# hangxu0304/DeepReduce

Measured on NVIDIA H100. Metric: ResNet-50 images/sec (whole job, device-timed, max over ranks), higher is better.
Workload: dtype bf16

## Files before the change

### deepreduce_b200/models/fused_bn.py

```python
from __future__ import annotations

import os

import torch
import torch.nn as nn
import torch.nn.functional as F


def enabled() -> bool:
    return os.environ.get("DR_FUSED_BN", "1") != "0"


def _eligible_x(x: torch.Tensor) -> bool:
    return (x.is_cuda and x.dtype == torch.bfloat16 and x.dim() == 4 and x.stride(1) == 1
            and x.is_contiguous(memory_format=torch.channels_last) and x.size(1) % 8 == 0 and x.size(1) <= 8192
            and x.numel() < 2 ** 31 - 1 and x.numel() // x.size(1) > 1)


def _eligible_bn(bn: nn.BatchNorm2d) -> bool:
    return (bn.training and bn.track_running_stats and bn.running_mean is not None and bn.momentum is not None
            and bn.affine)


def eligible(x: torch.Tensor, bn: nn.BatchNorm2d) -> bool:
    return enabled() and _eligible_x(x) and _eligible_bn(bn)


def _stats(x, bn):
    from .. import ops
    bn.num_batches_tracked.add_(1)
    return ops.cuda_module().bn_stats(x, bn.running_mean, bn.running_var, float(bn.momentum), float(bn.eps))


def _grad(go):
    return go.contiguous(memory_format=torch.channels_last)


class _BNReLU(torch.autograd.Function):
    @staticmethod
    def forward(ctx, x, weight, bias, mean, invstd):
        from .. import ops
        y, mask = ops.cuda_module().bn_apply(0, x, [mean, invstd, weight, bias])
        ctx.save_for_backward(x, weight, mean, invstd, mask)
        return y

    @staticmethod
    def backward(ctx, gy):
        from .. import ops
        x, weight, mean, invstd, mask = ctx.saved_tensors
        dx, dw, db = ops.cuda_module().bn_backward(0, _grad(gy), mask, x, [mean, invstd, weight])
        return dx, dw, db, None, None


class _BNAddReLU(torch.autograd.Function):

    @staticmethod
    def forward(ctx, x, weight, bias, mean, invstd, z, wz, bz, mz, iz):
        from .. import ops
        mod = ops.cuda_module()
        if wz is None:
            o, mask = mod.bn_apply(1, x, [mean, invstd, weight, bias], z)
            ctx.save_for_backward(x, weight, mean, invstd, mask)
        else:
            o, mask = mod.bn_apply(2, x, [mean, invstd, weight, bias], z, [mz, iz, wz, bz])
            ctx.save_for_backward(x, weight, mean, invstd, mask, z, wz, mz, iz)
        ctx.has_bn_z = wz is not None
        return o

    @staticmethod
    def backward(ctx, go):
        from .. import ops
        mod = ops.cuda_module()
        saved = ctx.saved_tensors
        x, weight, mean, invstd, mask = saved[:5]
        if not ctx.has_bn_z:
            dx, dw, db, g = mod.bn_backward(1, _grad(go), mask, x, [mean, invstd, weight])
            return dx, dw, db, None, None, g, None, None, None, None
        z, wz, mz, iz = saved[5:]
        dx, dw, db, dz, dwz, dbz = mod.bn_backward(2, _grad(go), mask, x, [mean, invstd, weight], z, [mz, iz, wz])
        return dx, dw, db, None, None, dz, dwz, dbz, None, None


class _BNReLUMaxPool(torch.autograd.Function):

    @staticmethod
    def forward(ctx, x, weight, bias, mean, invstd):
        from .. import ops
        out, codes = ops.cuda_module().bn_apply_pool(x, [mean, invstd, weight, bias])
        ctx.save_for_backward(x, weight, mean, invstd, codes)
        return out

    @staticmethod
    def backward(ctx, go):
        from .. import ops
        x, weight, mean, invstd, codes = ctx.saved_tensors
        dx, dw, db = ops.cuda_module().bn_backward(3, _grad(go), codes, x, [mean, invstd, weight])
        return dx, dw, db, None, None


def _stem_pool(pool: nn.Module) -> bool:
    if type(pool) is not nn.MaxPool2d:
        return False
    pair = lambda v: tuple(v) if isinstance(v, (tuple, list)) else (v, v)
    return (pair(pool.kernel_size) == (3, 3) and pair(pool.stride) == (2, 2) and pair(pool.padding) == (1, 1)
            and pair(pool.dilation) == (1, 1) and not pool.ceil_mode and not pool.return_indices)


def bn_relu_maxpool(x: torch.Tensor, bn: nn.BatchNorm2d, pool: nn.MaxPool2d) -> torch.Tensor:
    if not (eligible(x, bn) and _stem_pool(pool)):
        return pool(F.relu(bn(x), inplace=True))
    mean, invstd = _stats(x, bn)
    return _BNReLUMaxPool.apply(x, bn.weight, bn.bias, mean, invstd)


def bn_relu(x: torch.Tensor, bn: nn.BatchNorm2d) -> torch.Tensor:
    if not eligible(x, bn):
        return F.relu(bn(x), inplace=True)
    mean, invstd = _stats(x, bn)
    return _BNReLU.apply(x, bn.weight, bn.bias, mean, invstd)


def bn_add_relu(x: torch.Tensor, bn: nn.BatchNorm2d, idt: torch.Tensor) -> torch.Tensor:
    if not (eligible(x, bn) and idt.dtype == x.dtype and idt.shape == x.shape and idt.stride() == x.stride()):
        return F.relu(bn(x) + idt, inplace=True)
    mean, invstd = _stats(x, bn)
    return _BNAddReLU.apply(x, bn.weight, bn.bias, mean, invstd, idt, None, None, None, None)


def bn_bn_add_relu(x: torch.Tensor, bn: nn.BatchNorm2d, xd: torch.Tensor, bnd: nn.BatchNorm2d) -> torch.Tensor:
    if not (eligible(x, bn) and eligible(xd, bnd) and xd.shape == x.shape and xd.stride() == x.stride()):
        return F.relu(bn(x) + bnd(xd), inplace=True)
    md, id_ = _stats(xd, bnd)
    mean, invstd = _stats(x, bn)
    return _BNAddReLU.apply(x, bn.weight, bn.bias, mean, invstd, xd, bnd.weight, bnd.bias, md, id_)
```

### deepreduce_b200/models/resnet.py

```python
from __future__ import annotations

import torch.nn as nn
import torch.nn.functional as F

from .fused_bn import bn_add_relu, bn_bn_add_relu, bn_relu, bn_relu_maxpool


class _BasicCifar(nn.Module):
    def __init__(self, inp, out, stride):
        super().__init__()
        self.conv1 = nn.Conv2d(inp, out, 3, stride, 1, bias=False)
        self.bn1 = nn.BatchNorm2d(out)
        self.conv2 = nn.Conv2d(out, out, 3, 1, 1, bias=False)
        self.bn2 = nn.BatchNorm2d(out)
        self.pad = None
        if stride != 1 or inp != out:
            self.pad = (out - inp, stride)

    def forward(self, x):
        y = F.relu(self.bn1(self.conv1(x)))
        y = self.bn2(self.conv2(y))
        if self.pad is not None:
            extra, s = self.pad
            x = F.pad(x[:, :, ::s, ::s], (0, 0, 0, 0, extra // 2, extra - extra // 2))
# ... 20 lines not shown
        return self.fc(x)


def resnet20(num_classes: int = 10) -> ResNetCifar:
    return ResNetCifar(3, num_classes)


class _Bottleneck(nn.Module):
    expansion = 4

    def __init__(self, inp, width, stride, downsample):
        super().__init__()
        out = width * self.expansion
        self.conv1 = nn.Conv2d(inp, width, 1, bias=False)
        self.bn1 = nn.BatchNorm2d(width)
        self.conv2 = nn.Conv2d(width, width, 3, stride, 1, bias=False)
        self.bn2 = nn.BatchNorm2d(width)
        self.conv3 = nn.Conv2d(width, out, 1, bias=False)
        self.bn3 = nn.BatchNorm2d(out)
        self.downsample = None
        if downsample:
            self.downsample = nn.Sequential(nn.Conv2d(inp, out, 1, stride, bias=False), nn.BatchNorm2d(out))

    def forward(self, x):
        xd = None if self.downsample is None else self.downsample[0](x)
        y = bn_relu(self.conv1(x), self.bn1)
        y = bn_relu(self.conv2(y), self.bn2)
        y = self.conv3(y)
        if xd is None:
            return bn_add_relu(y, self.bn3, x)
        return bn_bn_add_relu(y, self.bn3, xd, self.downsample[1])


class ResNet(nn.Module):
    def __init__(self, blocks=(3, 4, 6, 3), num_classes: int = 1000):
        super().__init__()
        self.conv1 = nn.Conv2d(3, 64, 7, 2, 3, bias=False)
        self.bn1 = nn.BatchNorm2d(64)
        self.maxpool = nn.MaxPool2d(3, 2, 1)
        stages, inp = [], 64
        for i, (n, width) in enumerate(zip(blocks, (64, 128, 256, 512))):
            for j in range(n):
                stride = 2 if (j == 0 and i > 0) else 1
                stages.append(_Bottleneck(inp, width, stride, downsample=(j == 0)))
                inp = width * 4
        self.layers = nn.Sequential(*stages)
        self.fc = nn.Linear(inp, num_classes)
        for m in self.modules():
            if isinstance(m, nn.Conv2d):
                nn.init.kaiming_normal_(m.weight, mode="fan_out", nonlinearity="relu")

    def forward(self, x):
        x = bn_relu_maxpool(self.conv1(x), self.bn1, self.maxpool)
        x = self.layers(x)
        x = F.adaptive_avg_pool2d(x, 1).flatten(1)
        return self.fc(x)


def resnet50(num_classes: int = 1000) -> ResNet:
    return ResNet((3, 4, 6, 3), num_classes)
```

### deepreduce_b200/ops/csrc/binding.cpp

```cpp
#include <ATen/cuda/CUDAContext.h>
#include <c10/cuda/CUDAGuard.h>
#include <c10/cuda/CUDAStream.h>
#include <torch/extension.h>

#include <condition_variable>
#include <deque>
#include <mutex>
#include <thread>

#include "ops.h"

namespace py = pybind11;
using dr::EngineParams;

#define CHECK_CUDA_T(x) TORCH_CHECK((x).is_cuda() && (x).is_contiguous(), #x " must be a contiguous CUDA tensor")

static cudaStream_t cur_stream() { return at::cuda::getCurrentCUDAStream().stream(); }

static void check_last(const char* what) {
  cudaError_t e = cudaGetLastError();
  TORCH_CHECK(e == cudaSuccess, what, ": ", cudaGetErrorString(e));
}

static torch::Tensor bloom_insert(torch::Tensor idx, int64_t k, int64_t m_bits, int64_t seed) {
// ... 296 lines not shown
              "bn_apply_pool: only kernel 3, stride 2, padding 1, dilation 1, floor mode");
  check_bn_input(x);
  const int64_t N = x.size(0), C = x.size(1), H = x.size(2), W = x.size(3);
  const dr::BnParams px = bn_params(p, C);
  c10::cuda::CUDAGuard g(x.device());
  const dr::PoolGeom pg{(int)H, (int)W, (int)((H - 1) / 2 + 1), (int)((W - 1) / 2 + 1)};
  auto out = torch::empty({N, C, pg.Ho, pg.Wo}, x.options().memory_format(at::MemoryFormat::ChannelsLast));
  auto codes = torch::empty({N * pg.Ho * pg.Wo, C}, x.options().dtype(torch::kUInt8));
  cudaError_t e = dr::launch_bn_apply_pool(x.data_ptr(), px, out.data_ptr(), codes.data_ptr(), (int)N, pg, (int)C,
                                           cur_stream());
  TORCH_CHECK(e == cudaSuccess, "bn_apply_pool: ", cudaGetErrorString(e));
  return {out, codes};
}

static dr::BnParams bn_bwd_params(const std::vector<torch::Tensor>& p, int64_t C) {
  TORCH_CHECK(p.size() == 3, "bn_backward: expected (mean, invstd, weight)");
  const char* names[3] = {"mean", "invstd", "weight"};
  for (int i = 0; i < 3; ++i) check_chan(p[i], C, names[i]);
  return {p[0].data_ptr<float>(), p[1].data_ptr<float>(), p[2].data_ptr<float>(), nullptr};
}

static std::vector<torch::Tensor> bn_backward(int64_t mode, torch::Tensor go, torch::Tensor mask, torch::Tensor x,
                                              std::vector<torch::Tensor> p, c10::optional<torch::Tensor> z,
                                              std::vector<torch::Tensor> pz) {
  TORCH_CHECK(mode >= 0 && mode <= 3, "bn_backward: mode must be 0, 1, 2 or 3");
  check_bn_input(x);
  const int64_t C = x.size(1), rows = x.numel() / C;
  dr::PoolGeom pg{(int)x.size(2), (int)x.size(3), (int)((x.size(2) - 1) / 2 + 1), (int)((x.size(3) - 1) / 2 + 1)};
  const std::vector<int64_t> go_shape =
      mode == 3 ? std::vector<int64_t>{x.size(0), C, pg.Ho, pg.Wo} : x.sizes().vec();
  TORCH_CHECK(go.sizes() == go_shape && go.scalar_type() == torch::kBFloat16 && go.device() == x.device() &&
                  go.is_contiguous(at::MemoryFormat::ChannelsLast),
              "bn_backward: go must be a channels_last bf16 tensor on x's device, of x's shape (mode 3: the pooled "
              "shape)");
  const int64_t mask_numel = mode == 3 ? go.numel() : rows * (C / 8);
  TORCH_CHECK(mask.is_cuda() && mask.scalar_type() == torch::kUInt8 && mask.is_contiguous() &&
                  mask.numel() == mask_numel && mask.device() == x.device(),
              "bn_backward: mask must be bn_apply's mask (mode 3: bn_apply_pool's codes) for x");
  c10::cuda::CUDAGuard guard(x.device());
  int block_y = 0, grid_y = 0;
  dr::bn_row_tree(rows, (int)C, &block_y, &grid_y);
  TORCH_CHECK((int64_t)block_y * grid_y <= rows, "bn_backward: reduction tree wider than the rows");
  const int n_sums = mode == 2 ? 3 : 2;
  auto f32 = x.options().dtype(torch::kFloat32);
  auto sums = torch::empty({n_sums, C}, f32);
  auto staging = grid_y > 1 ? torch::empty({n_sums, grid_y, C}, f32) : torch::Tensor();
  auto dx = torch::empty_like(x), dw = torch::empty({C}, f32), db = torch::empty({C}, f32);
  dr::BnBwd b{};
  b.go = go.data_ptr(); b.mask = mask.data_ptr<uint8_t>(); b.x = x.data_ptr();
  b.px = bn_bwd_params(p, C);
  b.dx = dx.data_ptr(); b.sums = sums.data_ptr<float>(); b.staging = grid_y > 1 ? staging.data_ptr<float>() : nullptr;
  b.dw = dw.data_ptr<float>(); b.db = db.data_ptr<float>();
  b.pool = pg;
  std::vector<torch::Tensor> res{dx, dw, db};
  torch::Tensor g;
  if (mode == 1 || mode == 3) {
    g = torch::empty_like(x);
    b.g = g.data_ptr();
    if (mode == 1) res.push_back(g);
  } else if (mode == 2) {
    TORCH_CHECK(z.has_value(), "bn_backward: mode 2 needs z");
    check_like_x(*z, x, "z");
    b.z = z->data_ptr();
    b.pz = bn_bwd_params(pz, C);
    auto dz = torch::empty_like(x), dwz = torch::empty({C}, f32), dbz = torch::empty({C}, f32);
    b.dz = dz.data_ptr(); b.dwz = dwz.data_ptr<float>(); b.dbz = dbz.data_ptr<float>();
    res.insert(res.end(), {dz, dwz, dbz});
  }
  cudaError_t e = dr::launch_bn_backward((int)mode, b, rows, (int)C, cur_stream());
  TORCH_CHECK(e == cudaSuccess, "bn_backward: ", cudaGetErrorString(e));
  return res;
}
// ... 201 lines not shown

PYBIND11_MODULE(TORCH_EXTENSION_NAME, m) {
  m.def("launch_count", [] { return (int64_t)dr::launch_count(); });
  m.def("bloom_insert", &bloom_insert);
  m.def("bloom_select", &bloom_select);
  m.def("qsgd_encode", &qsgd_encode);
  m.def("qsgd_decode", &qsgd_decode);
  m.def("pack_bits", &pack_bits);
  m.def("unpack_bits", &unpack_bits);
  m.def("polyfit_fit", &polyfit_fit);
  m.def("polyfit_eval", &polyfit_eval);
  m.def("dexp_fit", &dexp_fit);
  m.def("conflict_sets_pick", &conflict_sets_pick);
  m.def("delta_bp128_encode", &delta_bp128_encode);
  m.def("delta_bp128_decode", &delta_bp128_decode);
  m.def("u8_to_nhwc_norm", &u8_to_nhwc_norm);
  m.def("bn_stats", &bn_stats, py::arg("x"), py::arg("running_mean"), py::arg("running_var"), py::arg("momentum"),
        py::arg("eps"), py::arg("torch_kernel") = false);
  m.def("bn_apply", &bn_apply, py::arg("mode"), py::arg("x"), py::arg("p"), py::arg("z") = py::none(),
        py::arg("pz") = std::vector<torch::Tensor>{});
  m.def("bn_apply_pool", &bn_apply_pool, py::arg("x"), py::arg("p"), py::arg("kernel_size") = 3, py::arg("stride") = 2,
        py::arg("padding") = 1, py::arg("dilation") = 1, py::arg("ceil_mode") = false);
  m.def("bn_backward", &bn_backward, py::arg("mode"), py::arg("go"), py::arg("mask"), py::arg("x"), py::arg("p"),
        py::arg("z") = py::none(), py::arg("pz") = std::vector<torch::Tensor>{});
  m.def("rle_runs", &rle_runs);
  m.def("rle_indices", &rle_indices);
  m.def("arena_alloc", &arena_alloc);
  m.def("arena_free", [](int64_t p) { dr::arena_free((void*)p); });
  m.def("arena_export", &arena_export);
  m.def("arena_import", &arena_import);
  m.def("arena_close", [](int64_t p) { dr::arena_close((void*)p); });
  m.def("arena_as_tensor", &arena_as_tensor);
  m.def("enable_peer_access", [](std::vector<int> devices) { return dr::arena_enable_peer_access(devices.data(), (int)devices.size()); });
  m.attr("TILE") = dr::kTile;
  m.attr("ARENA_HDR_WORDS") = dr::kArenaHdrWords;
  m.attr("SLOT_HEADER_WORDS") = dr::kSlotHeaderWords;
  m.attr("HIST_BINS") = dr::kHistBins;
  m.attr("NUM_HIST") = dr::kNumHist;
  m.attr("PH_END") = (int)dr::kPhEnd;

  py::class_<Engine>(m, "Engine")
      .def(py::init<int64_t, int64_t, int64_t, int64_t, int64_t, int64_t, int64_t, int64_t, int64_t, int64_t, int64_t,
                    int64_t, int64_t, int64_t, std::vector<int64_t>, int, int>())
      .def("configure", &Engine::configure)
      .def("set_buffers", &Engine::set_buffers)
      .def("set_poly", &Engine::set_poly)
      .def("set_shard", &Engine::set_shard)
// ... 20 lines not shown
```

### deepreduce_b200/ops/csrc/bn.cu

```cuda
#include <cuda_bf16.h>

#include <algorithm>

#include "common.cuh"
#include "ops.h"

namespace dr {

namespace {

constexpr int kVec = 8;
constexpr int kApplyThreads = 256;
constexpr int kReduceThreads = 128;

struct ChanParams {
  float m[kVec], inv[kVec], w[kVec], b[kVec];
};

__device__ __forceinline__ void load8(const float* __restrict__ p, float* d) {
  const float4 a = __ldg(reinterpret_cast<const float4*>(p));
  const float4 b = __ldg(reinterpret_cast<const float4*>(p) + 1);
  d[0] = a.x; d[1] = a.y; d[2] = a.z; d[3] = a.w;
  d[4] = b.x; d[5] = b.y; d[6] = b.z; d[7] = b.w;
}

__device__ __forceinline__ void load_params(const BnParams& p, int c, ChanParams& o) {
  load8(p.mean + c, o.m);
  load8(p.invstd + c, o.inv);
  load8(p.weight + c, o.w);
  load8(p.bias + c, o.b);
}

__device__ __forceinline__ float bn_elem(float x, float m, float inv, float w, float b) {
  return __fmaf_rn(__fmul_rn(w, __fsub_rn(x, m)), inv, b);
}

__device__ __forceinline__ __nv_bfloat16 relu_bf16(__nv_bfloat16 v) {
  return __bfloat162float(v) <= 0.f ? __float2bfloat16_rn(0.f) : v;
}

template <int kMode>
__global__ void __launch_bounds__(kApplyThreads) bn_apply_kernel(const __nv_bfloat16* __restrict__ x, BnParams px,
                                                                 const __nv_bfloat16* __restrict__ z, BnParams pz,
                                                                 __nv_bfloat16* __restrict__ out,
                                                                 uint8_t* __restrict__ mask, int64_t rows, int C) {
  const int groups = C / kVec;
  const int rows_per_cta = blockDim.x / groups;
  const int rsub = threadIdx.x / groups;
  if (rsub >= rows_per_cta) return;
  const int c = (threadIdx.x % groups) * kVec;
  ChanParams a;
  load_params(px, c, a);
  ChanParams d;
  if (kMode == 2) load_params(pz, c, d);
  const int64_t step = (int64_t)gridDim.x * rows_per_cta;
#pragma unroll 2
  for (int64_t r = (int64_t)blockIdx.x * rows_per_cta + rsub; r < rows; r += step) {
    const int64_t off = r * C + c;
    const uint4 vx = *reinterpret_cast<const uint4*>(x + off);
    uint4 vz = make_uint4(0, 0, 0, 0);
    if (kMode != 0) vz = *reinterpret_cast<const uint4*>(z + off);
// ... 85 lines not shown
  uint4 g[4];
  uint2 code[4];
  int off;
  int nh, nw;
  int sh, sw;
};

__device__ __forceinline__ void pool_gather_codes(PoolGather& q, const uint8_t* __restrict__ codes, const PoolGeom& pg,
                                                  int row, int C, int c, bool valid) {
  const int w = row % pg.W, t = row / pg.W, h = t % pg.H, n = t / pg.H;
  const int ph = h >> 1, pw = w >> 1;
  q.nh = valid ? min((h + 1) / 2 + 1, pg.Ho) - ph : 0;
  q.nw = valid ? min((w + 1) / 2 + 1, pg.Wo) - pw : 0;
  q.sh = h - 2 * ph + 1;
  q.sw = w - 2 * pw + 1;
  q.off = ((n * pg.Ho + ph) * pg.Wo + pw) * C + c;
#pragma unroll
  for (int k = 0; k < 4; ++k) {
    const int a = k >> 1, b = k & 1;
    q.code[k] = a < q.nh && b < q.nw ? *reinterpret_cast<const uint2*>(codes + q.off + (a * pg.Wo + b) * C) : uint2{};
  }
}

__device__ __forceinline__ void pool_gather_grads(PoolGather& q, const __nv_bfloat16* __restrict__ gp,
                                                  const PoolGeom& pg, int C) {
#pragma unroll
  for (int k = 0; k < 4; ++k) {
    const int a = k >> 1, b = k & 1;
    q.g[k] = a < q.nh && b < q.nw ? *reinterpret_cast<const uint4*>(gp + q.off + (a * pg.Wo + b) * C) : uint4{};
  }
}

__device__ __forceinline__ void pool_gather_resolve(const PoolGather& q, uint4& g, unsigned& bits) {
  __nv_bfloat16* hg = reinterpret_cast<__nv_bfloat16*>(&g);
  const bool single = q.nh == 1 && q.nw == 1;
  bits = 0;
#pragma unroll
  for (int i = 0; i < kVec; ++i) {
    float s = 0.f;
    __nv_bfloat16 one = __float2bfloat16_rn(0.f);
    unsigned bit = 0;
#pragma unroll
    for (int k = 0; k < 4; ++k) {
      const int a = k >> 1, b = k & 1;
      const unsigned code = (reinterpret_cast<const uint8_t*>(&q.code[k]))[i];
      if (a < q.nh && b < q.nw && (int)(code & 0x7fu) == (q.sh - 2 * a) * 3 + (q.sw - 2 * b)) {
        const __nv_bfloat16 v = (reinterpret_cast<const __nv_bfloat16*>(&q.g[k]))[i];
        s = __fadd_rn(s, __bfloat162float(v));
        one = v;
        bit = code >> 7;
      }
    }
    hg[i] = single ? one : __float2bfloat16_rn(s);
    bits |= bit << i;
  }
}

__global__ void __launch_bounds__(kApplyThreads) bn_pool_grad_kernel(const __nv_bfloat16* __restrict__ gp,
                                                                     const uint8_t* __restrict__ codes,
                                                                     __nv_bfloat16* __restrict__ g, PoolGeom pg,
                                                                     int64_t rows, int C) {
  const int groups = C / kVec;
  const int rows_per_cta = blockDim.x / groups;
  const int rsub = threadIdx.x / groups;
  if (rsub >= rows_per_cta) return;
  const int c = (threadIdx.x % groups) * kVec;
  const int64_t step = (int64_t)gridDim.x * rows_per_cta;
#pragma unroll 2
  for (int64_t r = (int64_t)blockIdx.x * rows_per_cta + rsub; r < rows; r += step) {
    PoolGather q;
    pool_gather_codes(q, codes, pg, (int)r, C, c, true);
    pool_gather_grads(q, gp, pg, C);
    uint4 v;
    unsigned bits;
    pool_gather_resolve(q, v, bits);
    __nv_bfloat16* hv = reinterpret_cast<__nv_bfloat16*>(&v);
#pragma unroll
    for (int i = 0; i < kVec; ++i)
      if (!((bits >> i) & 1u)) hv[i] = __float2bfloat16_rn(0.f);
    *reinterpret_cast<uint4*>(g + r * C + c) = v;
  }
}

struct RowTree {
  int block_y, grid_y;
  __host__ __device__ int S() const { return block_y * grid_y; }
  __host__ __device__ int loops(int rows) const { return 1 + (rows - 1) / (S() * kLoads); }
  static constexpr int kLoads = 4;
};

constexpr int kStatsThreads = 256;

__device__ __forceinline__ void welford_update(float x, float inv, float valid, float& mean, float& m2n) {
  const float d0 = __fsub_rn(x, mean);
  mean = __fmaf_rn(d0, inv, mean);
// ... 165 lines not shown
}

struct BwdOut {
  float* sums;
  float* dw; float* db; float* dwz; float* dbz;
  float* staging;
};

__device__ __forceinline__ void bwd_store(const BwdOut& o, int k, int c, int C, float v, const float* invstd,
                                         const float* invstd_z) {
  o.sums[k * C + c] = v;
  if (k == 0) {
    o.db[c] = v;
    if (o.dbz) o.dbz[c] = v;
  } else if (k == 1) {
    o.dw[c] = __fmul_rn(v, invstd[c]);
  } else {
    o.dwz[c] = __fmul_rn(v, invstd_z[c]);
  }
}

__device__ __forceinline__ float masked(__nv_bfloat16 go, unsigned bit) { return bit ? __bfloat162float(go) : 0.f; }

template <int kMode>
__global__ void __launch_bounds__(kReduceThreads) bn_bwd_reduce_kernel(const __nv_bfloat16* __restrict__ go,
                                                                       const uint8_t* __restrict__ mask,
                                                                       const __nv_bfloat16* __restrict__ x,
                                                                       const float* __restrict__ mean,
                                                                       const float* __restrict__ invstd,
                                                                       const __nv_bfloat16* __restrict__ z,
                                                                       const float* __restrict__ mean_z,
                                                                       const float* __restrict__ invstd_z,
                                                                       __nv_bfloat16* __restrict__ g_out, BwdOut o,
                                                                       RowTree t, int rows, int C) {
  constexpr int kSums = kMode == 2 ? 3 : 2;
  constexpr int L = RowTree::kLoads;
  extern __shared__ float sh[];
  const int gpc = blockDim.x / t.block_y;
  const int tg = threadIdx.x % gpc, y = threadIdx.x / gpc;
  const int group = blockIdx.x * gpc + tg;
  const bool live = group * kVec < C;
  const int c = live ? group * kVec : 0;
  const int S = t.S();
  float m[kVec], mz[kVec];
#pragma unroll
  for (int i = 0; i < kVec; ++i) {
    m[i] = mean[c + i];
    mz[i] = kMode == 2 ? mean_z[c + i] : 0.f;
  }
  float acc[kSums][L][kVec];
#pragma unroll
  for (int k = 0; k < kSums; ++k)
#pragma unroll
    for (int j = 0; j < L; ++j)
#pragma unroll
      for (int i = 0; i < kVec; ++i) acc[k][j][i] = 0.f;
  const int mgroups = C / kVec;
  int r = blockIdx.y * t.block_y + y;
  const int n_loops = t.loops(rows);
  struct Batch {
    uint4 g[L], x[L], z[L];
    unsigned m[L];
  };
  auto load = [&](Batch& b, int r0) {
#pragma unroll
    for (int j = 0; j < L; ++j) {
      const int rr = r0 + j * S;
      if (live && rr < rows) {
        const int off = rr * C + c;
        b.g[j] = *reinterpret_cast<const uint4*>(go + off);
        b.x[j] = *reinterpret_cast<const uint4*>(x + off);
        if (kMode == 2) b.z[j] = *reinterpret_cast<const uint4*>(z + off);
        b.m[j] = kMode == 3 ? 0u : mask[rr * mgroups + group];
      } else {
        b.g[j] = uint4{}; b.x[j] = uint4{}; b.z[j] = uint4{}; b.m[j] = 0;
      }
    }
  };
  Batch cur;
  load(cur, r);
  for (int it = 0; it < n_loops; ++it) {
    Batch nxt;
    load(nxt, r + L * S);
    const unsigned* mb = cur.m;
#pragma unroll
    for (int j = 0; j < L; ++j) {
      const __nv_bfloat16* hg = reinterpret_cast<const __nv_bfloat16*>(&cur.g[j]);
      const __nv_bfloat16* hx = reinterpret_cast<const __nv_bfloat16*>(&cur.x[j]);
      const __nv_bfloat16* hz = reinterpret_cast<const __nv_bfloat16*>(&cur.z[j]);
      uint4 vo;
      __nv_bfloat16* ho = reinterpret_cast<__nv_bfloat16*>(&vo);
#pragma unroll
      for (int i = 0; i < kVec; ++i) {
        const unsigned bit = (mb[j] >> i) & 1u;
        const float g = kMode == 3 ? __bfloat162float(hg[i]) : masked(hg[i], bit);
        if (kMode == 1) ho[i] = bit ? hg[i] : __float2bfloat16_rn(0.f);
        acc[0][j][i] = __fadd_rn(acc[0][j][i], g);
        acc[1][j][i] = __fmaf_rn(__fsub_rn(__bfloat162float(hx[i]), m[i]), g, acc[1][j][i]);
        if (kMode == 2) acc[2][j][i] = __fmaf_rn(__fsub_rn(__bfloat162float(hz[i]), mz[i]), g, acc[2][j][i]);
      }
      if (kMode == 1 && live && r + j * S < rows) *reinterpret_cast<uint4*>(g_out + (r + j * S) * C + c) = vo;
    }
    cur = nxt;
    r += L * S;
  }
#pragma unroll
  for (int k = 0; k < kSums; ++k) {
#pragma unroll
    for (int i = 0; i < kVec; ++i)
#pragma unroll
      for (int j = 1; j < L; ++j) acc[k][0][i] = __fadd_rn(acc[k][0][i], acc[k][j][i]);
    tree_over_y<kVec>(acc[k][0], sh, y, t.block_y, tg * kVec, gpc * kVec);
  }
  if (y != 0 || !live) return;
#pragma unroll
  for (int k = 0; k < kSums; ++k)
#pragma unroll
    for (int i = 0; i < kVec; ++i) {
      if (t.grid_y > 1) o.staging[((size_t)k * t.grid_y + blockIdx.y) * C + c + i] = acc[k][0][i];
      else bwd_store(o, k, c + i, C, acc[k][0][i], invstd, invstd_z);
    }
}

__global__ void bn_bwd_finalize_kernel(BwdOut o, RowTree t, int n_sums, int C, const float* __restrict__ invstd,
                                       const float* __restrict__ invstd_z) {
  extern __shared__ float sh[];
// ... 18 lines not shown
  float inv[kVec], ww[kVec], sx[kVec];
  load8(mean + c, p.m);
  load8(invstd + c, inv);
  load8(w + c, ww);
  load8(sdy + c, p.sdy);
  load8(sxmu + c, sx);
#pragma unroll
  for (int i = 0; i < kVec; ++i) {
    p.f1[i] = __fmul_rn(__fmul_rn(__fmul_rn(inv[i], inv[i]), sx[i]), norm);
    p.f2[i] = __fmul_rn(ww[i], inv[i]);
  }
}

__device__ __forceinline__ __nv_bfloat16 elemt(float g, float x, const ElemtChan& p, int i, float norm) {
  const float a = __fmaf_rn(-p.sdy[i], norm, g);
  return __float2bfloat16_rn(__fmul_rn(__fmaf_rn(-p.f1[i], __fsub_rn(x, p.m[i]), a), p.f2[i]));
}

struct ElemtArgs {
  const float *mean, *invstd, *weight, *sums;
  const float *mean_z, *invstd_z, *weight_z;
};

template <int kMode>
__global__ void __launch_bounds__(kApplyThreads) bn_bwd_elemt_kernel(const __nv_bfloat16* __restrict__ g_in,
                                                                     const uint8_t* __restrict__ mask,
                                                                     const __nv_bfloat16* __restrict__ x,
                                                                     const __nv_bfloat16* __restrict__ z, ElemtArgs a,
                                                                     __nv_bfloat16* __restrict__ dx,
                                                                     __nv_bfloat16* __restrict__ dz, float norm,
                                                                     int64_t rows, int C) {
  const int groups = C / kVec;
  const int rows_per_cta = blockDim.x / groups;
  const int rsub = threadIdx.x / groups;
  if (rsub >= rows_per_cta) return;
  const int c = (threadIdx.x % groups) * kVec;
  ElemtChan p;
  elemt_params(a.mean, a.invstd, a.weight, a.sums, a.sums + C, norm, c, p);
  ElemtChan q;
  if (kMode == 2) elemt_params(a.mean_z, a.invstd_z, a.weight_z, a.sums, a.sums + 2 * C, norm, c, q);
  const int64_t step = (int64_t)gridDim.x * rows_per_cta;
#pragma unroll 2
  for (int64_t r = (int64_t)blockIdx.x * rows_per_cta + rsub; r < rows; r += step) {
    const int64_t off = r * C + c;
    const uint4 vg = *reinterpret_cast<const uint4*>(g_in + off);
    const unsigned mb = kMode == 1 || kMode == 3 ? 0xffu : mask[r * groups + c / kVec];
    const uint4 vx = *reinterpret_cast<const uint4*>(x + off);
    uint4 vz = make_uint4(0, 0, 0, 0);
    if (kMode == 2) vz = *reinterpret_cast<const uint4*>(z + off);
    const __nv_bfloat16* hg = reinterpret_cast<const __nv_bfloat16*>(&vg);
    const __nv_bfloat16* hx = reinterpret_cast<const __nv_bfloat16*>(&vx);
    const __nv_bfloat16* hz = reinterpret_cast<const __nv_bfloat16*>(&vz);
    uint4 vo, vd;
    __nv_bfloat16* ho = reinterpret_cast<__nv_bfloat16*>(&vo);
    __nv_bfloat16* hd = reinterpret_cast<__nv_bfloat16*>(&vd);
#pragma unroll
    for (int i = 0; i < kVec; ++i) {
      const float g = masked(hg[i], (mb >> i) & 1u);
      ho[i] = elemt(g, __bfloat162float(hx[i]), p, i, norm);
      if (kMode == 2) hd[i] = elemt(g, __bfloat162float(hz[i]), q, i, norm);
    }
    *reinterpret_cast<uint4*>(dx + off) = vo;
    if (kMode == 2) *reinterpret_cast<uint4*>(dz + off) = vd;
  }
}

__global__ void bn_update_stats_kernel(const float* __restrict__ mean, float* __restrict__ var_invstd,
                                       float* __restrict__ running_mean, float* __restrict__ running_var, int C,
// ... 29 lines not shown
  cudaError_t e = rows_grid(bn_apply_kernel<kMode>, rows, C, grid, threads);
  if (e != cudaSuccess) return e;
  count_launch();
  bn_apply_kernel<kMode><<<grid, threads, 0, st>>>(reinterpret_cast<const __nv_bfloat16*>(x), px,
                                                   reinterpret_cast<const __nv_bfloat16*>(z), pz,
                                                   reinterpret_cast<__nv_bfloat16*>(out),
                                                   reinterpret_cast<uint8_t*>(mask), rows, C);
  return cudaGetLastError();
}

int last_pow2(unsigned n) {
  n |= n >> 1; n |= n >> 2; n |= n >> 4; n |= n >> 8; n |= n >> 16;
  return std::max<int>(1, (int)(n - (n >> 1)));
}

RowTree row_tree(int rows, int C) {
  const int block_x = std::min(last_pow2((unsigned)C), 32);
  const int block_y = std::min(last_pow2((unsigned)((rows + 15) / 16)), 512 / block_x);
  int grid_y = std::min((rows + block_y * 16 - 1) / (block_y * 16), 128);
  if (grid_y < 8) grid_y = 1;
  return {block_y, grid_y};
}

template <int kMode>
cudaError_t launch_bwd_reduce(const BnBwd& b, const RowTree& t, const BwdOut& o, int rows, int C, cudaStream_t st) {
  const int groups = C / kVec;
  const int gpc = std::min(groups, std::max(1, kReduceThreads / t.block_y));
  const dim3 grid((groups + gpc - 1) / gpc, t.grid_y);
  const int threads = gpc * t.block_y;
  count_launch();
  bn_bwd_reduce_kernel<kMode><<<grid, threads, threads * kVec * sizeof(float), st>>>(
      reinterpret_cast<const __nv_bfloat16*>(b.go), b.mask, reinterpret_cast<const __nv_bfloat16*>(b.x), b.px.mean,
      b.px.invstd, reinterpret_cast<const __nv_bfloat16*>(b.z), b.pz.mean, b.pz.invstd,
      reinterpret_cast<__nv_bfloat16*>(b.g), o, t, rows, C);
  return cudaGetLastError();
}

template <int kMode>
cudaError_t launch_bwd_elemt(const BnBwd& b, const ElemtArgs& a, int64_t rows, int C, cudaStream_t st) {
  int grid = 0, threads = 0;
  cudaError_t e = rows_grid(bn_bwd_elemt_kernel<kMode>, rows, C, grid, threads);
  if (e != cudaSuccess) return e;
  const float norm = (float)(1.0 / (double)rows);
  count_launch();
  bn_bwd_elemt_kernel<kMode><<<grid, threads, 0, st>>>(
      reinterpret_cast<const __nv_bfloat16*>(kMode == 1 || kMode == 3 ? b.g : b.go), b.mask,
      reinterpret_cast<const __nv_bfloat16*>(b.x), reinterpret_cast<const __nv_bfloat16*>(b.z), a,
      reinterpret_cast<__nv_bfloat16*>(b.dx), reinterpret_cast<__nv_bfloat16*>(b.dz), norm, rows, C);
  return cudaGetLastError();
}

template <int kMode>
cudaError_t launch_backward(const BnBwd& b, int64_t rows64, int C, cudaStream_t st) {
  const int rows = (int)rows64;
  const RowTree t = row_tree(rows, C);
  const BwdOut o{b.sums, b.dw, b.db, b.dwz, b.dbz, b.staging};
  cudaError_t e;
  if (kMode == 3) {
    int grid = 0, threads = 0;
    e = rows_grid(bn_pool_grad_kernel, rows64, C, grid, threads);
    if (e != cudaSuccess) return e;
    count_launch();
    bn_pool_grad_kernel<<<grid, threads, 0, st>>>(reinterpret_cast<const __nv_bfloat16*>(b.go), b.mask,
                                                  reinterpret_cast<__nv_bfloat16*>(b.g), b.pool, rows64, C);
    e = cudaGetLastError();
    if (e != cudaSuccess) return e;
  }
  BnBwd bb = b;
  if (kMode == 3) bb.go = b.g;
  e = launch_bwd_reduce<kMode>(bb, t, o, rows, C, st);
  if (e != cudaSuccess) return e;
  if (t.grid_y > 1) {
    const int cols = std::max(1, 512 / t.block_y);
    const int threads = cols * t.block_y;
    count_launch();
    bn_bwd_finalize_kernel<<<(C + cols - 1) / cols, threads, threads * sizeof(float), st>>>(
        o, t, kMode == 2 ? 3 : 2, C, b.px.invstd, b.pz.invstd);
    e = cudaGetLastError();
    if (e != cudaSuccess) return e;
  }
  const ElemtArgs a{b.px.mean, b.px.invstd, b.px.weight, b.sums, b.pz.mean, b.pz.invstd, b.pz.weight};
  return launch_bwd_elemt<kMode>(b, a, rows64, C, st);
}

cudaError_t launch_stats(const BnStats& s, int rows, int C, cudaStream_t st) {
  const RowTree t = row_tree(rows, C);
  const int grid_y = t.grid_y;
  const StatsOut o{s.mean, s.invstd, s.running_mean, s.running_var,
                   s.staging, s.staging + (size_t)grid_y * C, reinterpret_cast<int*>(s.staging + 2 * (size_t)grid_y * C),
                   s.momentum, s.bessel, s.eps};
  const int groups = C / kVec;
  const int gpc = std::min(groups, std::max(1, kStatsThreads / (RowTree::kLoads * t.block_y)));
  const int threads = gpc * RowTree::kLoads * t.block_y;
  count_launch();
  bn_stats_kernel<<<dim3((groups + gpc - 1) / gpc, grid_y), threads, WelfordSlots<kVec>::bytes(threads), st>>>(
      reinterpret_cast<const __nv_bfloat16*>(s.x), o, t, rows, C);
  cudaError_t e = cudaGetLastError();
  if (e != cudaSuccess || grid_y == 1) return e;
  const int cols = std::max(1, 512 / t.block_y);
  const int fthreads = cols * t.block_y;
  count_launch();
  bn_stats_finalize_kernel<<<(C + cols - 1) / cols, fthreads, WelfordSlots<1>::bytes(fthreads), st>>>(o, t, C);
  return cudaGetLastError();
}

}

void bn_row_tree(int64_t rows, int C, int* block_y, int* grid_y) {
  const RowTree t = row_tree((int)rows, C);
  *block_y = t.block_y;
  *grid_y = t.grid_y;
}

cudaError_t launch_bn_backward(int mode, const BnBwd& b, int64_t rows, int C, cudaStream_t st) {
  if (rows == 0) return cudaSuccess;
  switch (mode) {
    case 0: return launch_backward<0>(b, rows, C, st);
    case 1: return launch_backward<1>(b, rows, C, st);
    case 2: return launch_backward<2>(b, rows, C, st);
    case 3: return launch_backward<3>(b, rows, C, st);
    default: return cudaErrorInvalidValue;
  }
}

cudaError_t launch_bn_stats(const BnStats& s, int64_t rows, int C, cudaStream_t st) {
  if (rows == 0) return cudaSuccess;
  return launch_stats(s, (int)rows, C, st);
}

cudaError_t launch_bn_update_stats(const float* mean, float* var_invstd, float* running_mean, float* running_var, int C,
                                   float momentum, float bessel, float eps, cudaStream_t st) {
  count_launch();
  bn_update_stats_kernel<<<(C + 255) / 256, 256, 0, st>>>(mean, var_invstd, running_mean, running_var, C, momentum,
                                                          bessel, eps);
  return cudaGetLastError();
}

cudaError_t launch_bn_apply(int mode, const void* x, const BnParams& px, const void* z, const BnParams& pz, void* out,
                            void* mask, int64_t rows, int C, cudaStream_t st) {
  switch (mode) {
    case 0: return launch_apply<0>(x, px, z, pz, out, mask, rows, C, st);
    case 1: return launch_apply<1>(x, px, z, pz, out, mask, rows, C, st);
    case 2: return launch_apply<2>(x, px, z, pz, out, mask, rows, C, st);
// ... 20 lines not shown
```

### deepreduce_b200/ops/csrc/ops.h

```cpp
#pragma once
#include <cuda_runtime.h>
#include <stdint.h>

#include "plan.h"

namespace dr {

int engine_max_grid(int blocks_per_sm, int dyn_smem_bytes);
cudaError_t engine_launch(const EngineParams& P, int grid, int blocks_per_sm, int dyn_smem_bytes, cudaStream_t stream);
void count_launch(int n);
long long launch_count();

void launch_bloom_insert(const int64_t* idx, int64_t n, uint32_t* filter, uint32_t n_hash, uint32_t m_bits,
                         uint32_t seed, cudaStream_t st);
void launch_bloom_count(const uint32_t* filter, uint32_t d, uint32_t n_hash, uint32_t m_bits, uint32_t seed,
                        uint32_t* tile_counts, uint32_t* tile_excl, cudaStream_t st);
void launch_bloom_emit(const uint32_t* filter, uint32_t d, uint32_t n_hash, uint32_t m_bits, uint32_t seed,
                       const uint32_t* tile_excl, int64_t* out, uint32_t limit, cudaStream_t st);
void launch_qsgd_encode(const float* v, int64_t K, int bucket, int q, uint32_t seed, void* lvl, bool i16, float* norms,
                        cudaStream_t st);
void launch_qsgd_decode(const void* lvl, bool i16, const float* norms, int64_t K, int bucket, int q, float* out,
                        cudaStream_t st);
void launch_pack_bits(const int64_t* vals, int64_t n, int bits, uint32_t* out, int64_t n_words, cudaStream_t st);
void launch_unpack_bits(const uint32_t* in, int64_t n_words, int64_t n, int bits, int64_t* out, cudaStream_t st);
// ... 21 lines not shown
void* arena_import(const ArenaHandle& h);
void arena_close(void* p);
int arena_enable_peer_access(const int* devices, int n);
void launch_u8_to_nhwc_norm(const uint8_t* in, void* out_bf16, int64_t n_pix, const float* mean, const float* inv_std,
                            cudaStream_t st);

struct BnParams { const float* mean; const float* invstd; const float* weight; const float* bias; };
void bn_row_tree(int64_t rows, int C, int* block_y, int* grid_y);
struct BnStats {
  const void* x;
  float* mean; float* invstd; float* running_mean; float* running_var;
  float* staging;
  float momentum, bessel, eps;
};
cudaError_t launch_bn_stats(const BnStats& s, int64_t rows, int C, cudaStream_t st);
cudaError_t launch_bn_update_stats(const float* mean, float* var_invstd, float* running_mean, float* running_var, int C,
                                   float momentum, float bessel, float eps, cudaStream_t st);
cudaError_t launch_bn_apply(int mode, const void* x, const BnParams& px, const void* z, const BnParams& pz, void* out,
                            void* mask, int64_t rows, int C, cudaStream_t st);
struct PoolGeom { int H, W, Ho, Wo; };
cudaError_t launch_bn_apply_pool(const void* x, const BnParams& px, void* out, void* codes, int N, const PoolGeom& pg,
                                 int C, cudaStream_t st);
struct BnBwd {
  const void* go; const uint8_t* mask; const void* x; const void* z;
  BnParams px, pz;
  void* dx; void* dz; void* g;
  float* sums; float* staging; float* dw; float* db; float* dwz; float* dbz;
  PoolGeom pool;
};
cudaError_t launch_bn_backward(int mode, const BnBwd& b, int64_t rows, int C, cudaStream_t st);

}
```

Measured before the change: 5947.

## Fuse residual-branch gradient accumulation into fused BN backward kernels

Fused BN outputs that feed both the next block's main path and its skip connection now return two autograd outputs (the output and a detached alias). The two incoming gradients are summed inside the BN backward reduce, elementwise and pool-grad kernels instead of by autograd's separate accumulation add. This removes one elementwise add kernel and its extra read/write traffic per identity block in backward. In exchange it loads a second gradient tensor in the kernels and drops the look-ahead prefetch in the mode-2 reduce path, which may lower its memory-level parallelism.

```diff
diff --git a/deepreduce_b200/models/fused_bn.py b/deepreduce_b200/models/fused_bn.py
--- a/deepreduce_b200/models/fused_bn.py
+++ b/deepreduce_b200/models/fused_bn.py
@@ -36,6 +36,18 @@
     return go.contiguous(memory_format=torch.channels_last)
 
 
+def _fork(ctx, o, fork):
+    if not fork:
+        return o
+    ctx.set_materialize_grads(False)
+    return o, o.detach()
+
+
+def _grads(grads):
+    gs = [_grad(g) for g in grads if g is not None]
+    return (gs + [None, None])[:2]
+
+
 class _BNReLU(torch.autograd.Function):
     @staticmethod
     def forward(ctx, x, weight, bias, mean, invstd):
@@ -55,7 +67,7 @@
 class _BNAddReLU(torch.autograd.Function):
 
     @staticmethod
-    def forward(ctx, x, weight, bias, mean, invstd, z, wz, bz, mz, iz):
+    def forward(ctx, x, weight, bias, mean, invstd, z, wz, bz, mz, iz, fork):
         from .. import ops
         mod = ops.cuda_module()
         if wz is None:
@@ -65,37 +77,43 @@
             o, mask = mod.bn_apply(2, x, [mean, invstd, weight, bias], z, [mz, iz, wz, bz])
             ctx.save_for_backward(x, weight, mean, invstd, mask, z, wz, mz, iz)
         ctx.has_bn_z = wz is not None
-        return o
+        return _fork(ctx, o, fork)
 
     @staticmethod
-    def backward(ctx, go):
+    def backward(ctx, *grads):
         from .. import ops
         mod = ops.cuda_module()
+        go, go2 = _grads(grads)
+        if go is None:
+            return (None,) * 11
         saved = ctx.saved_tensors
         x, weight, mean, invstd, mask = saved[:5]
         if not ctx.has_bn_z:
-            dx, dw, db, g = mod.bn_backward(1, _grad(go), mask, x, [mean, invstd, weight])
-            return dx, dw, db, None, None, g, None, None, None, None
+            dx, dw, db, g = mod.bn_backward(1, go, mask, x, [mean, invstd, weight], go2=go2)
+            return dx, dw, db, None, None, g, None, None, None, None, None
         z, wz, mz, iz = saved[5:]
-        dx, dw, db, dz, dwz, dbz = mod.bn_backward(2, _grad(go), mask, x, [mean, invstd, weight], z, [mz, iz, wz])
-        return dx, dw, db, None, None, dz, dwz, dbz, None, None
+        dx, dw, db, dz, dwz, dbz = mod.bn_backward(2, go, mask, x, [mean, invstd, weight], z, [mz, iz, wz], go2=go2)
+        return dx, dw, db, None, None, dz, dwz, dbz, None, None, None
 
 
 class _BNReLUMaxPool(torch.autograd.Function):
 
     @staticmethod
-    def forward(ctx, x, weight, bias, mean, invstd):
+    def forward(ctx, x, weight, bias, mean, invstd, fork):
         from .. import ops
         out, codes = ops.cuda_module().bn_apply_pool(x, [mean, invstd, weight, bias])
         ctx.save_for_backward(x, weight, mean, invstd, codes)
-        return out
+        return _fork(ctx, out, fork)
 
     @staticmethod
-    def backward(ctx, go):
+    def backward(ctx, *grads):
         from .. import ops
+        go, go2 = _grads(grads)
+        if go is None:
+            return (None,) * 6
         x, weight, mean, invstd, codes = ctx.saved_tensors
-        dx, dw, db = ops.cuda_module().bn_backward(3, _grad(go), codes, x, [mean, invstd, weight])
-        return dx, dw, db, None, None
+        dx, dw, db = ops.cuda_module().bn_backward(3, go, codes, x, [mean, invstd, weight], go2=go2)
+        return dx, dw, db, None, None, None
 
 
 def _stem_pool(pool: nn.Module) -> bool:
@@ -106,11 +124,15 @@
             and pair(pool.dilation) == (1, 1) and not pool.ceil_mode and not pool.return_indices)
 
 
-def bn_relu_maxpool(x: torch.Tensor, bn: nn.BatchNorm2d, pool: nn.MaxPool2d) -> torch.Tensor:
+def _pair(o, fork):
+    return (o, o) if fork else o
+
+
+def bn_relu_maxpool(x: torch.Tensor, bn: nn.BatchNorm2d, pool: nn.MaxPool2d, fork: bool = False):
     if not (eligible(x, bn) and _stem_pool(pool)):
-        return pool(F.relu(bn(x), inplace=True))
+        return _pair(pool(F.relu(bn(x), inplace=True)), fork)
     mean, invstd = _stats(x, bn)
-    return _BNReLUMaxPool.apply(x, bn.weight, bn.bias, mean, invstd)
+    return _BNReLUMaxPool.apply(x, bn.weight, bn.bias, mean, invstd, fork)
 
 
 def bn_relu(x: torch.Tensor, bn: nn.BatchNorm2d) -> torch.Tensor:
@@ -120,16 +142,16 @@
     return _BNReLU.apply(x, bn.weight, bn.bias, mean, invstd)
 
 
-def bn_add_relu(x: torch.Tensor, bn: nn.BatchNorm2d, idt: torch.Tensor) -> torch.Tensor:
+def bn_add_relu(x: torch.Tensor, bn: nn.BatchNorm2d, idt: torch.Tensor, fork: bool = False):
     if not (eligible(x, bn) and idt.dtype == x.dtype and idt.shape == x.shape and idt.stride() == x.stride()):
-        return F.relu(bn(x) + idt, inplace=True)
+        return _pair(F.relu(bn(x) + idt, inplace=True), fork)
     mean, invstd = _stats(x, bn)
-    return _BNAddReLU.apply(x, bn.weight, bn.bias, mean, invstd, idt, None, None, None, None)
+    return _BNAddReLU.apply(x, bn.weight, bn.bias, mean, invstd, idt, None, None, None, None, fork)
 
 
-def bn_bn_add_relu(x: torch.Tensor, bn: nn.BatchNorm2d, xd: torch.Tensor, bnd: nn.BatchNorm2d) -> torch.Tensor:
+def bn_bn_add_relu(x: torch.Tensor, bn: nn.BatchNorm2d, xd: torch.Tensor, bnd: nn.BatchNorm2d, fork: bool = False):
     if not (eligible(x, bn) and eligible(xd, bnd) and xd.shape == x.shape and xd.stride() == x.stride()):
-        return F.relu(bn(x) + bnd(xd), inplace=True)
+        return _pair(F.relu(bn(x) + bnd(xd), inplace=True), fork)
     md, id_ = _stats(xd, bnd)
     mean, invstd = _stats(x, bn)
-    return _BNAddReLU.apply(x, bn.weight, bn.bias, mean, invstd, xd, bnd.weight, bnd.bias, md, id_)
+    return _BNAddReLU.apply(x, bn.weight, bn.bias, mean, invstd, xd, bnd.weight, bnd.bias, md, id_, fork)
diff --git a/deepreduce_b200/models/resnet.py b/deepreduce_b200/models/resnet.py
--- a/deepreduce_b200/models/resnet.py
+++ b/deepreduce_b200/models/resnet.py
@@ -66,14 +66,16 @@
         if downsample:
             self.downsample = nn.Sequential(nn.Conv2d(inp, out, 1, stride, bias=False), nn.BatchNorm2d(out))
 
-    def forward(self, x):
-        xd = None if self.downsample is None else self.downsample[0](x)
+    def forward(self, x, skip=None, fork=False):
+        skip = x if skip is None else skip
+        xd = None if self.downsample is None else self.downsample[0](skip)
         y = bn_relu(self.conv1(x), self.bn1)
         y = bn_relu(self.conv2(y), self.bn2)
         y = self.conv3(y)
         if xd is None:
-            return bn_add_relu(y, self.bn3, x)
-        return bn_bn_add_relu(y, self.bn3, xd, self.downsample[1])
+            return bn_add_relu(y, self.bn3, skip, fork=fork)
+        o = bn_bn_add_relu(y, self.bn3, xd, self.downsample[1])
+        return (o, None) if fork else o
 
 
 class ResNet(nn.Module):
@@ -95,8 +97,9 @@
                 nn.init.kaiming_normal_(m.weight, mode="fan_out", nonlinearity="relu")
 
     def forward(self, x):
-        x = bn_relu_maxpool(self.conv1(x), self.bn1, self.maxpool)
-        x = self.layers(x)
+        x, skip = bn_relu_maxpool(self.conv1(x), self.bn1, self.maxpool), None
+        for blk in self.layers:
+            x, skip = blk(x, skip, fork=True)
         x = F.adaptive_avg_pool2d(x, 1).flatten(1)
         return self.fc(x)
 
diff --git a/deepreduce_b200/ops/csrc/binding.cpp b/deepreduce_b200/ops/csrc/binding.cpp
--- a/deepreduce_b200/ops/csrc/binding.cpp
+++ b/deepreduce_b200/ops/csrc/binding.cpp
@@ -342,17 +342,19 @@
 
 static std::vector<torch::Tensor> bn_backward(int64_t mode, torch::Tensor go, torch::Tensor mask, torch::Tensor x,
                                               std::vector<torch::Tensor> p, c10::optional<torch::Tensor> z,
-                                              std::vector<torch::Tensor> pz) {
+                                              std::vector<torch::Tensor> pz, c10::optional<torch::Tensor> go2) {
   TORCH_CHECK(mode >= 0 && mode <= 3, "bn_backward: mode must be 0, 1, 2 or 3");
+  TORCH_CHECK(!go2.has_value() || mode != 0, "bn_backward: mode 0 takes no go2");
   check_bn_input(x);
   const int64_t C = x.size(1), rows = x.numel() / C;
   dr::PoolGeom pg{(int)x.size(2), (int)x.size(3), (int)((x.size(2) - 1) / 2 + 1), (int)((x.size(3) - 1) / 2 + 1)};
   const std::vector<int64_t> go_shape =
       mode == 3 ? std::vector<int64_t>{x.size(0), C, pg.Ho, pg.Wo} : x.sizes().vec();
-  TORCH_CHECK(go.sizes() == go_shape && go.scalar_type() == torch::kBFloat16 && go.device() == x.device() &&
-                  go.is_contiguous(at::MemoryFormat::ChannelsLast),
-              "bn_backward: go must be a channels_last bf16 tensor on x's device, of x's shape (mode 3: the pooled "
-              "shape)");
+  for (const torch::Tensor* t : {&go, go2.has_value() ? &*go2 : &go})
+    TORCH_CHECK(t->sizes() == go_shape && t->scalar_type() == torch::kBFloat16 && t->device() == x.device() &&
+                    t->is_contiguous(at::MemoryFormat::ChannelsLast),
+                "bn_backward: go and go2 must be channels_last bf16 tensors on x's device, of x's shape (mode 3: the "
+                "pooled shape)");
   const int64_t mask_numel = mode == 3 ? go.numel() : rows * (C / 8);
   TORCH_CHECK(mask.is_cuda() && mask.scalar_type() == torch::kUInt8 && mask.is_contiguous() &&
                   mask.numel() == mask_numel && mask.device() == x.device(),
@@ -367,7 +369,7 @@
   auto staging = grid_y > 1 ? torch::empty({n_sums, grid_y, C}, f32) : torch::Tensor();
   auto dx = torch::empty_like(x), dw = torch::empty({C}, f32), db = torch::empty({C}, f32);
   dr::BnBwd b{};
-  b.go = go.data_ptr(); b.mask = mask.data_ptr<uint8_t>(); b.x = x.data_ptr();
+  b.go = go.data_ptr(); b.go2 = go2.has_value() ? go2->data_ptr() : nullptr; b.mask = mask.data_ptr<uint8_t>(); b.x = x.data_ptr();
   b.px = bn_bwd_params(p, C);
   b.dx = dx.data_ptr(); b.sums = sums.data_ptr<float>(); b.staging = grid_y > 1 ? staging.data_ptr<float>() : nullptr;
   b.dw = dw.data_ptr<float>(); b.db = db.data_ptr<float>();
@@ -615,7 +617,7 @@
   m.def("bn_apply_pool", &bn_apply_pool, py::arg("x"), py::arg("p"), py::arg("kernel_size") = 3, py::arg("stride") = 2,
         py::arg("padding") = 1, py::arg("dilation") = 1, py::arg("ceil_mode") = false);
   m.def("bn_backward", &bn_backward, py::arg("mode"), py::arg("go"), py::arg("mask"), py::arg("x"), py::arg("p"),
-        py::arg("z") = py::none(), py::arg("pz") = std::vector<torch::Tensor>{});
+        py::arg("z") = py::none(), py::arg("pz") = std::vector<torch::Tensor>{}, py::arg("go2") = py::none());
   m.def("rle_runs", &rle_runs);
   m.def("rle_indices", &rle_indices);
   m.def("arena_alloc", &arena_alloc);
diff --git a/deepreduce_b200/ops/csrc/bn.cu b/deepreduce_b200/ops/csrc/bn.cu
--- a/deepreduce_b200/ops/csrc/bn.cu
+++ b/deepreduce_b200/ops/csrc/bn.cu
@@ -37,6 +37,16 @@
 
 __device__ __forceinline__ __nv_bfloat16 relu_bf16(__nv_bfloat16 v) {
   return __bfloat162float(v) <= 0.f ? __float2bfloat16_rn(0.f) : v;
+}
+
+__device__ __forceinline__ uint4 add_bf16x8(const uint4& a, const uint4& b) {
+  uint4 s;
+  const __nv_bfloat16* ha = reinterpret_cast<const __nv_bfloat16*>(&a);
+  const __nv_bfloat16* hb = reinterpret_cast<const __nv_bfloat16*>(&b);
+  __nv_bfloat16* hs = reinterpret_cast<__nv_bfloat16*>(&s);
+#pragma unroll
+  for (int i = 0; i < kVec; ++i) hs[i] = __float2bfloat16_rn(__fadd_rn(__bfloat162float(ha[i]), __bfloat162float(hb[i])));
+  return s;
 }
 
 template <int kMode>
@@ -168,12 +178,16 @@
   }
 }
 
+template <bool kTwo>
 __device__ __forceinline__ void pool_gather_grads(PoolGather& q, const __nv_bfloat16* __restrict__ gp,
-                                                  const PoolGeom& pg, int C) {
+                                                  const __nv_bfloat16* __restrict__ gp2, const PoolGeom& pg, int C) {
 #pragma unroll
   for (int k = 0; k < 4; ++k) {
     const int a = k >> 1, b = k & 1;
-    q.g[k] = a < q.nh && b < q.nw ? *reinterpret_cast<const uint4*>(gp + q.off + (a * pg.Wo + b) * C) : uint4{};
+    const bool in = a < q.nh && b < q.nw;
+    const int off = q.off + (a * pg.Wo + b) * C;
+    q.g[k] = in ? *reinterpret_cast<const uint4*>(gp + off) : uint4{};
+    if (kTwo && in) q.g[k] = add_bf16x8(q.g[k], *reinterpret_cast<const uint4*>(gp2 + off));
   }
 }
 
@@ -202,7 +216,9 @@
   }
 }
 
+template <bool kTwo>
 __global__ void __launch_bounds__(kApplyThreads) bn_pool_grad_kernel(const __nv_bfloat16* __restrict__ gp,
+                                                                     const __nv_bfloat16* __restrict__ gp2,
                                                                      const uint8_t* __restrict__ codes,
                                                                      __nv_bfloat16* __restrict__ g, PoolGeom pg,
                                                                      int64_t rows, int C) {
@@ -216,7 +232,7 @@
   for (int64_t r = (int64_t)blockIdx.x * rows_per_cta + rsub; r < rows; r += step) {
     PoolGather q;
     pool_gather_codes(q, codes, pg, (int)r, C, c, true);
-    pool_gather_grads(q, gp, pg, C);
+    pool_gather_grads<kTwo>(q, gp, gp2, pg, C);
     uint4 v;
     unsigned bits;
     pool_gather_resolve(q, v, bits);
@@ -428,8 +444,9 @@
 
 __device__ __forceinline__ float masked(__nv_bfloat16 go, unsigned bit) { return bit ? __bfloat162float(go) : 0.f; }
 
-template <int kMode>
+template <int kMode, bool kTwo>
 __global__ void __launch_bounds__(kReduceThreads) bn_bwd_reduce_kernel(const __nv_bfloat16* __restrict__ go,
+                                                                       const __nv_bfloat16* __restrict__ go2,
                                                                        const uint8_t* __restrict__ mask,
                                                                        const __nv_bfloat16* __restrict__ x,
                                                                        const float* __restrict__ mean,
@@ -464,8 +481,9 @@
   const int mgroups = C / kVec;
   int r = blockIdx.y * t.block_y + y;
   const int n_loops = t.loops(rows);
+  constexpr bool kAhead = !(kTwo && kMode == 2);
   struct Batch {
-    uint4 g[L], x[L], z[L];
+    uint4 g[L], g2[L], x[L], z[L];
     unsigned m[L];
   };
   auto load = [&](Batch& b, int r0) {
@@ -475,19 +493,25 @@
       if (live && rr < rows) {
         const int off = rr * C + c;
         b.g[j] = *reinterpret_cast<const uint4*>(go + off);
+        if (kTwo) b.g2[j] = *reinterpret_cast<const uint4*>(go2 + off);
         b.x[j] = *reinterpret_cast<const uint4*>(x + off);
         if (kMode == 2) b.z[j] = *reinterpret_cast<const uint4*>(z + off);
         b.m[j] = kMode == 3 ? 0u : mask[rr * mgroups + group];
       } else {
-        b.g[j] = uint4{}; b.x[j] = uint4{}; b.z[j] = uint4{}; b.m[j] = 0;
+        b.g[j] = uint4{}; b.g2[j] = uint4{}; b.x[j] = uint4{}; b.z[j] = uint4{}; b.m[j] = 0;
       }
     }
   };
   Batch cur;
-  load(cur, r);
+  if (kAhead) load(cur, r);
   for (int it = 0; it < n_loops; ++it) {
+    if (!kAhead) load(cur, r);
+    if (kTwo) {
+#pragma unroll
+      for (int j = 0; j < L; ++j) cur.g[j] = add_bf16x8(cur.g[j], cur.g2[j]);
+    }
     Batch nxt;
-    load(nxt, r + L * S);
+    if (kAhead) load(nxt, r + L * S);
     const unsigned* mb = cur.m;
 #pragma unroll
     for (int j = 0; j < L; ++j) {
@@ -507,7 +531,7 @@
       }
       if (kMode == 1 && live && r + j * S < rows) *reinterpret_cast<uint4*>(g_out + (r + j * S) * C + c) = vo;
     }
-    cur = nxt;
+    if (kAhead) cur = nxt;
     r += L * S;
   }
 #pragma unroll
@@ -572,8 +596,9 @@
   const float *mean_z, *invstd_z, *weight_z;
 };
 
-template <int kMode>
+template <int kMode, bool kTwo>
 __global__ void __launch_bounds__(kApplyThreads) bn_bwd_elemt_kernel(const __nv_bfloat16* __restrict__ g_in,
+                                                                     const __nv_bfloat16* __restrict__ g2_in,
                                                                      const uint8_t* __restrict__ mask,
                                                                      const __nv_bfloat16* __restrict__ x,
                                                                      const __nv_bfloat16* __restrict__ z, ElemtArgs a,
@@ -593,7 +618,8 @@
 #pragma unroll 2
   for (int64_t r = (int64_t)blockIdx.x * rows_per_cta + rsub; r < rows; r += step) {
     const int64_t off = r * C + c;
-    const uint4 vg = *reinterpret_cast<const uint4*>(g_in + off);
+    uint4 vg = *reinterpret_cast<const uint4*>(g_in + off);
+    if (kTwo) vg = add_bf16x8(vg, *reinterpret_cast<const uint4*>(g2_in + off));
     const unsigned mb = kMode == 1 || kMode == 3 ? 0xffu : mask[r * groups + c / kVec];
     const uint4 vx = *reinterpret_cast<const uint4*>(x + off);
     uint4 vz = make_uint4(0, 0, 0, 0);
@@ -669,35 +695,36 @@
   return {block_y, grid_y};
 }
 
-template <int kMode>
+template <int kMode, bool kTwo>
 cudaError_t launch_bwd_reduce(const BnBwd& b, const RowTree& t, const BwdOut& o, int rows, int C, cudaStream_t st) {
   const int groups = C / kVec;
   const int gpc = std::min(groups, std::max(1, kReduceThreads / t.block_y));
   const dim3 grid((groups + gpc - 1) / gpc, t.grid_y);
   const int threads = gpc * t.block_y;
   count_launch();
-  bn_bwd_reduce_kernel<kMode><<<grid, threads, threads * kVec * sizeof(float), st>>>(
-      reinterpret_cast<const __nv_bfloat16*>(b.go), b.mask, reinterpret_cast<const __nv_bfloat16*>(b.x), b.px.mean,
-      b.px.invstd, reinterpret_cast<const __nv_bfloat16*>(b.z), b.pz.mean, b.pz.invstd,
-      reinterpret_cast<__nv_bfloat16*>(b.g), o, t, rows, C);
+  bn_bwd_reduce_kernel<kMode, kTwo><<<grid, threads, threads * kVec * sizeof(float), st>>>(
+      reinterpret_cast<const __nv_bfloat16*>(b.go), reinterpret_cast<const __nv_bfloat16*>(b.go2), b.mask,
+      reinterpret_cast<const __nv_bfloat16*>(b.x), b.px.mean, b.px.invstd, reinterpret_cast<const __nv_bfloat16*>(b.z),
+      b.pz.mean, b.pz.invstd, reinterpret_cast<__nv_bfloat16*>(b.g), o, t, rows, C);
   return cudaGetLastError();
 }
 
-template <int kMode>
+template <int kMode, bool kTwo>
 cudaError_t launch_bwd_elemt(const BnBwd& b, const ElemtArgs& a, int64_t rows, int C, cudaStream_t st) {
   int grid = 0, threads = 0;
-  cudaError_t e = rows_grid(bn_bwd_elemt_kernel<kMode>, rows, C, grid, threads);
+  cudaError_t e = rows_grid(bn_bwd_elemt_kernel<kMode, kTwo>, rows, C, grid, threads);
   if (e != cudaSuccess) return e;
   const float norm = (float)(1.0 / (double)rows);
   count_launch();
-  bn_bwd_elemt_kernel<kMode><<<grid, threads, 0, st>>>(
-      reinterpret_cast<const __nv_bfloat16*>(kMode == 1 || kMode == 3 ? b.g : b.go), b.mask,
-      reinterpret_cast<const __nv_bfloat16*>(b.x), reinterpret_cast<const __nv_bfloat16*>(b.z), a,
-      reinterpret_cast<__nv_bfloat16*>(b.dx), reinterpret_cast<__nv_bfloat16*>(b.dz), norm, rows, C);
+  bn_bwd_elemt_kernel<kMode, kTwo><<<grid, threads, 0, st>>>(
+      reinterpret_cast<const __nv_bfloat16*>(kMode == 1 || kMode == 3 ? b.g : b.go),
+      reinterpret_cast<const __nv_bfloat16*>(b.go2), b.mask, reinterpret_cast<const __nv_bfloat16*>(b.x),
+      reinterpret_cast<const __nv_bfloat16*>(b.z), a, reinterpret_cast<__nv_bfloat16*>(b.dx),
+      reinterpret_cast<__nv_bfloat16*>(b.dz), norm, rows, C);
   return cudaGetLastError();
 }
 
-template <int kMode>
+template <int kMode, bool kTwo>
 cudaError_t launch_backward(const BnBwd& b, int64_t rows64, int C, cudaStream_t st) {
   const int rows = (int)rows64;
   const RowTree t = row_tree(rows, C);
@@ -705,17 +732,18 @@
   cudaError_t e;
   if (kMode == 3) {
     int grid = 0, threads = 0;
-    e = rows_grid(bn_pool_grad_kernel, rows64, C, grid, threads);
+    e = rows_grid(bn_pool_grad_kernel<kTwo>, rows64, C, grid, threads);
     if (e != cudaSuccess) return e;
     count_launch();
-    bn_pool_grad_kernel<<<grid, threads, 0, st>>>(reinterpret_cast<const __nv_bfloat16*>(b.go), b.mask,
-                                                  reinterpret_cast<__nv_bfloat16*>(b.g), b.pool, rows64, C);
+    bn_pool_grad_kernel<kTwo><<<grid, threads, 0, st>>>(reinterpret_cast<const __nv_bfloat16*>(b.go),
+                                                        reinterpret_cast<const __nv_bfloat16*>(b.go2), b.mask,
+                                                        reinterpret_cast<__nv_bfloat16*>(b.g), b.pool, rows64, C);
     e = cudaGetLastError();
     if (e != cudaSuccess) return e;
   }
   BnBwd bb = b;
   if (kMode == 3) bb.go = b.g;
-  e = launch_bwd_reduce<kMode>(bb, t, o, rows, C, st);
+  e = launch_bwd_reduce<kMode, kTwo && kMode != 3>(bb, t, o, rows, C, st);
   if (e != cudaSuccess) return e;
   if (t.grid_y > 1) {
     const int cols = std::max(1, 512 / t.block_y);
@@ -727,7 +755,7 @@
     if (e != cudaSuccess) return e;
   }
   const ElemtArgs a{b.px.mean, b.px.invstd, b.px.weight, b.sums, b.pz.mean, b.pz.invstd, b.pz.weight};
-  return launch_bwd_elemt<kMode>(b, a, rows64, C, st);
+  return launch_bwd_elemt<kMode, kTwo && kMode == 2>(b, a, rows64, C, st);
 }
 
 cudaError_t launch_stats(const BnStats& s, int rows, int C, cudaStream_t st) {
@@ -761,11 +789,12 @@
 
 cudaError_t launch_bn_backward(int mode, const BnBwd& b, int64_t rows, int C, cudaStream_t st) {
   if (rows == 0) return cudaSuccess;
+  const bool two = b.go2 != nullptr;
   switch (mode) {
-    case 0: return launch_backward<0>(b, rows, C, st);
-    case 1: return launch_backward<1>(b, rows, C, st);
-    case 2: return launch_backward<2>(b, rows, C, st);
-    case 3: return launch_backward<3>(b, rows, C, st);
+    case 0: return two ? cudaErrorInvalidValue : launch_backward<0, false>(b, rows, C, st);
+    case 1: return two ? launch_backward<1, true>(b, rows, C, st) : launch_backward<1, false>(b, rows, C, st);
+    case 2: return two ? launch_backward<2, true>(b, rows, C, st) : launch_backward<2, false>(b, rows, C, st);
+    case 3: return two ? launch_backward<3, true>(b, rows, C, st) : launch_backward<3, false>(b, rows, C, st);
     default: return cudaErrorInvalidValue;
   }
 }
diff --git a/deepreduce_b200/ops/csrc/ops.h b/deepreduce_b200/ops/csrc/ops.h
--- a/deepreduce_b200/ops/csrc/ops.h
+++ b/deepreduce_b200/ops/csrc/ops.h
@@ -67,7 +67,7 @@
 cudaError_t launch_bn_apply_pool(const void* x, const BnParams& px, void* out, void* codes, int N, const PoolGeom& pg,
                                  int C, cudaStream_t st);
 struct BnBwd {
-  const void* go; const uint8_t* mask; const void* x; const void* z;
+  const void* go; const void* go2; const uint8_t* mask; const void* x; const void* z;
   BnParams px, pz;
   void* dx; void* dz; void* g;
   float* sums; float* staging; float* dw; float* db; float* dwz; float* dbz;
```

After: 6161 (median of 6 runs). 3.6% higher.
